# arancormonk/dsd-neo

Measured on AMD Instinct MI355X. Metric: I/Q Msamples/s end-to-end (demod->FEC->MBE) per GPU; % HBM roofline, higher is better.
Workload: dtype f32

## Files before the change

### dsd-neo_amd/csrc/ddn_api_chain.cpp

```cpp
#include <hip/hip_runtime.h>
#include <hsa/hsa.h>
#include <hsa/hsa_ext_amd.h>

#include <condition_variable>
#include <cstdio>
#include <cstdlib>
#include <cstring>
#include <deque>
#include <mutex>
#include <new>
#include <thread>

#include "ddn_api_util.h"
#include "ddn_chain.h"
#include "ddn_device.h"
#include "ddn_hip.h"
#include "ddn_internal.h"
#include "ddn_mbe.h"

enum { NSET = 3 };
static inline int
set_prev(int cur) {
    return (cur + NSET - 1) % NSET;
}
// ... 18 lines not shown
    float* d_pcm_dense[NSET] = {nullptr, nullptr, nullptr};
    int32_t *d_pcm_slot[NSET] = {nullptr, nullptr, nullptr}, *d_pcm_bcnt = nullptr, *d_pcm_boff = nullptr,
            *d_pcm_total[NSET] = {nullptr, nullptr, nullptr};
    int32_t *d_new[NSET], *d_ev[NSET], *d_nev[NSET], *d_evd[NSET];
    int32_t *d_evl[NSET], *d_evdl[NSET], *d_nevl[NSET];
    int32_t *d_cnt_scan, *d_cnt_full[NSET];
    int32_t* d_nid[NSET];
    int32_t *d_lists, *d_list_n;
    uint8_t* d_cls;
    uint8_t *d_tsbk[NSET], *d_tsbk_crc;
    uint8_t *d_words[2], *d_wrel, *d_werrs, *d_vldu;
    uint8_t *d_rs_d[2], *d_rs_p[2], *d_rs_st[2];
    uint8_t *d_lsd, *d_lsd_ok;
    int16_t* d_lsd_llr;
    uint8_t *d_hdu_hex, *d_hdu_par, *d_hdu_st, *d_hdu_d, *d_hdu_p, *d_hdu_rs;
    uint8_t *d_td_d, *d_td_p, *d_td_st, *d_td_rd, *d_td_rp, *d_td_rs;
    int PF, PB;
    int32_t *d_pdu_slot, *d_pdu_info, *d_n_pdu, *d_pdu_metric;
    uint8_t *d_pdu_hdr, *d_pdu_valid, *d_pdu_blocks, *d_pdu_wanted, *d_pdu_cand, *d_pdu_blocks18, *d_pdu_crc9;
    int32_t* d_pdu_cnt;
    int16_t *d_pdu_llr, *d_pdu_hllr;
    int64_t* d_first;
    int32_t *d_sc, *d_nldu, *d_sc_out, *d_imbe_res, *d_res_out;
    uint8_t *d_imbe_fr, *d_imbe_soft, *d_imbe_fl, *d_imbe_d;
    float* d_pcm[NSET];
    hipStream_t s_main, s_aux, s_copy, s_copy2;
    hipStream_t s_voice = nullptr;
    hipEvent_t ev_fork = nullptr, ev_join = nullptr;
    hipEvent_t ev_produced[NSET], ev_consumed[NSET], ev_out[NSET];
    hipEvent_t ev_in[2], ev_in_free[2];
    hipEvent_t ev_loop[NSET] = {nullptr, nullptr, nullptr};
    hipEvent_t ev_pre[NSET] = {nullptr, nullptr, nullptr}, ev_join_a = nullptr, ev_aux_done[NSET] = {nullptr, nullptr, nullptr};
    int synth_beside_loop = 1;
    int have_deferred = 0, deferred_set = 0, deferred_dense = 0;
    int want_rec2 = 0;
    ddn_p25_chain_host_out pending_out;
    int have_pending = 0, pending_set = 0;
    int sdma = 0;
    hsa_agent_t sdma_gpu, sdma_cpu;
    uint32_t sdma_engine = 0;
    hsa_signal_t sdma_sig[NSET];
    int sdma_sig_ok = 0;
    struct OutJob {
        int set;
        ddn_p25_chain_host_out out;
    };
// ... 173 lines not shown
        c->stride = (size_t)c->T + c->ms;
        c->S = (size_t)c->B * (size_t)c->F;
        c->V = (size_t)c->B * (size_t)c->Fv * 9;
        const size_t B = (size_t)c->B, S = c->S, V = c->V;
        DdnPool& m = c->pool;
        bool ok = m.alloc(&c->d_disc, B * (size_t)c->n) && m.alloc(&c->d_sym_cnt, B);
        for (int k = 0; k < NSET && ok; k++) {
            ok = m.alloc(&c->d_rec[k], B * c->stride * 10) && m.alloc(&c->d_fl[k], B * c->stride) && m.alloc(&c->d_new[k], B)
                 && m.alloc(&c->d_ev[k], B * (size_t)c->E * 4) && m.alloc(&c->d_nev[k], B) && m.alloc(&c->d_evd[k], B * (size_t)c->E * 4)
                 && m.alloc(&c->d_evl[k], B * (size_t)c->EL * 4) && m.alloc(&c->d_evdl[k], B * (size_t)c->EL * 4) && m.alloc(&c->d_nevl[k], B)
                 && m.alloc(&c->d_cnt_full[k], B) && m.alloc(&c->d_nid[k], S * 4) && m.alloc(&c->d_tsbk[k], 3 * S * 12) && m.alloc(&c->d_pcm[k], V * 160);
        }
        ok = ok && m.alloc(&c->d_cnt_scan, B) && m.alloc(&c->d_cls, S) && m.alloc(&c->d_lists, S * DDN_LIST_COUNT) && m.alloc(&c->d_list_n, 8)
             && m.alloc(&c->d_tsbk_crc, 3 * S) && m.alloc(&c->d_words[0], S * 240)
             && m.alloc(&c->d_words[1], S * 240) && m.alloc(&c->d_wrel, S * 240) && m.alloc(&c->d_werrs, S * 24) && m.alloc(&c->d_vldu, S)
             && m.alloc(&c->d_rs_d[0], S * 72) && m.alloc(&c->d_rs_d[1], S * 96) && m.alloc(&c->d_rs_p[0], S * 72)
             && m.alloc(&c->d_rs_p[1], S * 48) && m.alloc(&c->d_rs_st[0], S) && m.alloc(&c->d_rs_st[1], S) && m.alloc(&c->d_lsd, S * 32)
             && m.alloc(&c->d_lsd_ok, S * 2) && m.alloc(&c->d_lsd_llr, S * 32) && m.alloc(&c->d_hdu_hex, S * 216)
             && m.alloc(&c->d_hdu_par, S * 432) && m.alloc(&c->d_hdu_st, S * 36) && m.alloc(&c->d_hdu_d, S * 120)
             && m.alloc(&c->d_hdu_p, S * 96) && m.alloc(&c->d_hdu_rs, S) && m.alloc(&c->d_td_d, S * 144) && m.alloc(&c->d_td_p, S * 144)
             && m.alloc(&c->d_td_st, S * 12) && m.alloc(&c->d_td_rd, S * 72) && m.alloc(&c->d_td_rp, S * 72) && m.alloc(&c->d_td_rs, S)
             && m.alloc(&c->d_first, V) && m.alloc(&c->d_sc, V) && m.alloc(&c->d_nldu, B) && m.alloc(&c->d_sc_out, V)
             && m.alloc(&c->d_imbe_res, V * 5) && m.alloc(&c->d_res_out, V * 5) && m.alloc(&c->d_imbe_fr, V * 184)
             && m.alloc(&c->d_imbe_soft, V * 368) && m.alloc(&c->d_imbe_fl, V) && m.alloc(&c->d_imbe_d, V * 88)
             && m.alloc(&c->d_pdu_slot, B * (size_t)c->PF) && m.alloc(&c->d_pdu_info, B * (size_t)c->PF * 4)
             && m.alloc(&c->d_n_pdu, B) && m.alloc(&c->d_pdu_hdr, B * (size_t)c->PF * 12)
             && m.alloc(&c->d_pdu_valid, B * (size_t)c->PF * (size_t)c->PB) && m.alloc(&c->d_pdu_blocks, B * (size_t)c->PF * (size_t)c->PB * 12)
             && m.alloc(&c->d_pdu_metric, B * (size_t)c->PF * (size_t)c->PB) && m.alloc(&c->d_pdu_llr, B * (size_t)c->PF * (size_t)c->PB * 196)
             && m.alloc(&c->d_pdu_wanted, B * (size_t)c->PF * (size_t)c->PB) && m.alloc(&c->d_pdu_cand, B * (size_t)c->PF * (size_t)c->PB * 8 * 24)
             && m.alloc(&c->d_pdu_blocks18, B * (size_t)c->PF * (size_t)c->PB * 18) && m.alloc(&c->d_pdu_crc9, B * (size_t)c->PF * (size_t)c->PB)
             && m.alloc(&c->d_pdu_cnt, B * (size_t)c->PF * (size_t)c->PB) && m.alloc(&c->d_pdu_hllr, B * (size_t)c->PF * 196);
        if (!ok) {
            ddn_set_error("ddn_p25_chain_create: device allocation failed");
            rc = DDN_ENOMEM;
            break;
        }
        if (hipStreamCreateWithPriority(&c->s_main, hipStreamNonBlocking, -1) != hipSuccess
            || hipStreamCreateWithFlags(&c->s_aux, hipStreamNonBlocking) != hipSuccess
            || hipStreamCreateWithFlags(&c->s_copy, hipStreamNonBlocking) != hipSuccess
            || hipStreamCreateWithFlags(&c->s_copy2, hipStreamNonBlocking) != hipSuccess
            || hipStreamCreateWithFlags(&c->s_voice, hipStreamNonBlocking) != hipSuccess
            || hipEventCreateWithFlags(&c->ev_fork, hipEventDisableTiming) != hipSuccess
            || hipEventCreateWithFlags(&c->ev_join, hipEventDisableTiming) != hipSuccess
            || hipEventCreateWithFlags(&c->ev_user, hipEventDisableTiming) != hipSuccess) {
            rc = DDN_EHIP;
            break;
        }
// ... 479 lines not shown
        HIP_TRY(ddn_dev_chain_pdu_gather(rec, c->d_cnt_full[cur], stride, d_sp, c->d_pdu_slot, c->d_pdu_info, c->B, c->F, c->PF, c->PB,
                                         c->d_pdu_llr, c->d_pdu_valid, st));
        HIP_TRY(ddn_dev_p25_half_rate_list_wanted(c->d_pdu_llr, (int)NB, 8, c->d_pdu_valid, (uint32_t*)c->d_pdu_cand, c->d_pdu_cnt, st));
        HIP_TRY(ddn_dev_chain_pdu_take_first(c->d_pdu_cand, c->d_pdu_cnt, (int)NB, c->d_pdu_blocks, c->d_pdu_metric, st));
        HIP_TRY(ddn_dev_chain_pdu_r34_wanted(c->d_pdu_slot, c->d_pdu_hdr, c->d_pdu_info, c->d_pdu_valid, (int)NB, c->PB, c->d_pdu_wanted, st));
        DDN_TRY(ddn_fec_p25_mbf34_list_batch(c->d_pdu_llr, NB, 8, c->d_pdu_wanted, (ddn_p25_mbf34_candidate*)c->d_pdu_cand, c->d_pdu_cnt, st));
        HIP_TRY(ddn_dev_chain_pdu_r34_select(c->d_pdu_cand, c->d_pdu_cnt, c->d_pdu_wanted, (int)NB, c->d_pdu_blocks18, c->d_pdu_crc9, st));
        HIP_TRY(ddn_dev_chain_pdu_combine(rec, c->d_cnt_full[cur], stride, d_sp, c->d_pdu_slot, c->d_pdu_info, c->d_pdu_llr, c->d_pdu_valid,
                                          c->d_pdu_blocks, (int)NE, c->PF, c->PB, c->d_pdu_hllr, c->d_pdu_wanted, st));
        HIP_TRY(ddn_dev_p25_half_rate_list_wanted(c->d_pdu_hllr, (int)NE, 8, c->d_pdu_wanted, (uint32_t*)c->d_pdu_cand, c->d_pdu_cnt, st));
        HIP_TRY(ddn_dev_chain_pdu_finish(c->d_pdu_slot, c->d_pdu_blocks, c->d_pdu_valid, c->d_pdu_blocks18, c->d_pdu_cand, c->d_pdu_cnt,
                                         c->d_pdu_wanted, (int)NE, c->PB, c->d_pdu_hdr, c->d_pdu_info, st));
    }
    if (c->lp.MB > 0) {
        DDN_TRY(chain_long_pdu(c, cur, flush, st));
    }
    if (c->timing) {
        HIP_TRY(hipEventRecord(c->ev_t[4], st));
    }
    if (c->want_rec2) {
        HIP_TRY(ddn_dev_chain_pack2(c->d_rec[cur], c->d_fl[cur], (size_t)c->B * c->stride, c->d_rec2[cur], vst));
        c->want_rec2 = 0;
    }
    DDN_TRY(ddn_p25p1_framer_voice_index(c->fr, c->d_nid[cur], c->d_cnt_full[cur], c->Fv, stride, c->d_first, c->d_sc, c->d_nldu, vst));
    DDN_TRY(ddn_p25p1_imbe_deinterleave_batch(rec, (size_t)c->B * stride, c->d_first, c->d_sc, V, c->d_imbe_fr, c->d_imbe_soft,
                                              c->d_imbe_fl, c->d_sc_out, vst));
    DDN_TRY(ddn_mbe_frame_decode_batch(DDN_MBE_IMBE_7200X4400, c->d_imbe_fr, nullptr, V, c->d_imbe_d, c->d_imbe_res, vst));
    DDN_TRY(ddn_mbe_result_skip_batch(c->d_imbe_fl, V, c->d_imbe_res, vst));
    if (ev_pre) {
        if (vst != st) {
            HIP_TRY(hipEventRecord(c->ev_join_a, vst));
            HIP_TRY(hipStreamWaitEvent(st, c->ev_join_a, 0));
        }
        HIP_TRY(hipEventRecord(ev_pre, st));
    }
    if (defer_synth && vst != st && ev_pre && c->cfg.vocoder) {
        DDN_TRY(ddn_mbe_params_only(c->mbe, c->d_imbe_d, c->d_imbe_res, (size_t)c->Fv * 9, c->d_res_out, vst));
        HIP_TRY(hipEventRecord(c->ev_join_a, vst));
        HIP_TRY(hipStreamWaitEvent(st, c->ev_join_a, 0));
        HIP_TRY(hipEventRecord(ev_pre, st));
        c->have_deferred = 1;
        c->deferred_set = cur;
        c->deferred_dense = 0;
        return DDN_OK;
    }
    if (c->cfg.vocoder) {
        DDN_TRY(ddn_mbe_synth_batch(c->mbe, c->d_imbe_d, c->d_imbe_res, (size_t)c->Fv * 9, c->d_pcm[cur], c->d_res_out, vst));
    }
    if (vst != st) {
        HIP_TRY(hipEventRecord(c->ev_join, vst));
        HIP_TRY(hipStreamWaitEvent(st, c->ev_join, 0));
// ... 521 lines not shown
```

### dsd-neo_amd/csrc/ddn_api_framer.cpp

```cpp

#include <hip/hip_runtime.h>

#include <cstring>
#include <new>

#include "ddn_api_util.h"
#include "ddn_device.h"
#include "ddn_internal.h"

enum { T_NID = 0, T_BLK0, T_BLK1, T_BLK2, T_LDU1, T_LDU2, T_HDU_HEX, T_HDU_PAR, T_TDULC_DATA, T_TDULC_PAR, T_LSD, T_COUNT };

struct ddn_p25p1_framer {
    int n_channels, max_frames;
    int32_t* d_sync_pos;
    int32_t* d_n_syncs;
    int32_t* d_dropped;
    int32_t* d_tab[T_COUNT];
    int n_off[T_COUNT], max_off[T_COUNT];
    int32_t *d_first9, *d_status9;
    DdnPool pool;
};

extern "C" int
ddn_p25p1_framer_create(int n_channels, int max_frames_per_channel, ddn_p25p1_framer** out) {
// ... 172 lines not shown
    if (!f || !d_first_record || !d_status_count) {
        ddn_set_error("ddn_p25p1_framer_imbe_index: null argument");
        return DDN_EINVAL;
    }
    HIP_TRY(ddn_dev_imbe_index(f->d_sync_pos, f->d_n_syncs, f->n_channels, f->max_frames, max_symbols, f->d_first9,
                               f->d_status9, d_first_record, d_status_count, (hipStream_t)hip_stream));
    return DDN_OK;
}

extern "C" int
ddn_p25p1_framer_voice_index(ddn_p25p1_framer* f, const int32_t* d_nid4, const int32_t* d_counts, int max_ldu_per_channel, size_t max_symbols,
                             int64_t* d_first_record, int32_t* d_status_count, int32_t* d_n_ldu, void* hip_stream) {
    if (!f || !d_nid4 || !d_counts || max_ldu_per_channel <= 0 || !d_first_record || !d_status_count) {
        ddn_set_error("ddn_p25p1_framer_voice_index: bad argument");
        return DDN_EINVAL;
    }
    HIP_TRY(ddn_dev_voice_index(f->d_sync_pos, f->d_n_syncs, d_nid4, d_counts, f->n_channels, f->max_frames, max_ldu_per_channel,
                                max_symbols, f->d_first9, f->d_status9, d_first_record, d_status_count, d_n_ldu,
                                (hipStream_t)hip_stream));
    return DDN_OK;
}

extern "C" int
ddn_p25p1_framer_pack_ldu_rs(ddn_p25p1_framer* f, int ldu, const uint8_t* d_words240, uint8_t* d_data_bits,
                             uint8_t* d_parity_bits, void* hip_stream) {
    if (!f || (ldu != 1 && ldu != 2) || !d_words240 || !d_data_bits || !d_parity_bits) {
        ddn_set_error("ddn_p25p1_framer_pack_ldu_rs: bad argument");
        return DDN_EINVAL;
    }
    HIP_TRY(ddn_dev_rs_pack(d_words240, (long)f->n_channels * f->max_frames, 24, 10, ldu == 1 ? 12 : 16, d_data_bits,
                            d_parity_bits, (hipStream_t)hip_stream));
    return DDN_OK;
}

extern "C" int
ddn_p25p1_framer_gather_hdu(ddn_p25p1_framer* f, const uint8_t* d_records10, const int32_t* d_counts, size_t max_symbols,
                            uint8_t* d_hex_bits216, uint8_t* d_parity_bits432, int16_t* d_hex_llr216,
                            int16_t* d_parity_llr432, uint8_t* d_valid, void* hip_stream) {
    if (!d_hex_bits216 || !d_parity_bits432) {
        ddn_set_error("ddn_p25p1_framer_gather_hdu: null argument");
        return DDN_EINVAL;
    }
    int rc = gather(f, T_HDU_HEX, d_records10, d_counts, max_symbols, d_hex_bits216, nullptr, d_hex_llr216, 216, 0,
                    nullptr, nullptr, nullptr, hip_stream);
    if (rc != DDN_OK) {
        return rc;
// ... 57 lines not shown
```

### dsd-neo_amd/csrc/ddn_device.h

```cpp
#ifndef DDN_DEVICE_H
#define DDN_DEVICE_H

#include <hip/hip_runtime.h>
#include <stddef.h>
#include <stdint.h>

#include "ddn_internal.h"

#ifdef DDN_EXPERIMENTS
#include <stdlib.h>
#define DDN_EXP_ENV(name) getenv(name)
#else
#define DDN_EXP_ENV(name) ((const char*)0)
#endif

#define DDN_TILE 256
#define DDN_DEFAULT_GROUP 8
#define DDN_CARRY_LEN 72

typedef struct DdnFskState {
    float prev_i, prev_q;
    int have_prev;
    float dc_est, peak_est;
} DdnFskState;
// ... 230 lines not shown
hipError_t ddn_dev_rs63_soft(uint8_t* data6, const uint8_t* parity6, const uint8_t* data_rel, const uint8_t* parity_rel,
                             int n_par, int n_data, int t, int threshold, int n, uint8_t* status, hipStream_t st);
hipError_t ddn_dev_rs63(uint8_t* data6, const uint8_t* parity6, int n_par, int n_data, int t, int n, uint8_t* status,
                        hipStream_t st);
hipError_t ddn_dev_hamming_10_6_3(uint8_t* bits10, int n, uint8_t* errs, hipStream_t st);
hipError_t ddn_dev_p25_crc16(const uint8_t* bytes, int item_bytes, int n, uint8_t* ok, hipStream_t st);
hipError_t ddn_dev_p25_lsd(uint8_t* bits16, const int16_t* llr16, int n, uint8_t* ok, hipStream_t st);
hipError_t ddn_dev_iq_cond_disc(const void* in, long n, size_t stride, int block_len, int n_channels,
                                const DdnIqCondConfig* cfg, DdnFskState* fsk, DdnIqCondState* cond, float* out,
                                size_t out_stride, hipStream_t st);
hipError_t ddn_dev_find_syncs(const uint8_t* flags, const int32_t* counts, int n_channels, size_t max_sym, int max_frames,
                              int32_t* sync_pos, int32_t* n_syncs, int32_t* dropped, hipStream_t st);
hipError_t ddn_dev_gather_fields(const uint8_t* rec, size_t max_sym, const int32_t* counts, const int32_t* sync_pos,
                                 const int32_t* n_syncs, int n_channels, int max_frames, const int32_t* offsets, int n_off,
                                 int max_off, uint8_t* bits, uint8_t* rel, int16_t* llr, int stride, int split_last,
                                 uint8_t* last_bit, uint8_t* last_rel, uint8_t* valid, uint8_t* dibits,
                                 uint8_t* dibit_rel, hipStream_t st);
hipError_t ddn_dev_rs_pack(const uint8_t* words, long n_slots, int n_words, int wstride, int n_data, uint8_t* data,
                           uint8_t* parity, hipStream_t st);
hipError_t ddn_dev_tdulc_rs_pack(const uint8_t* words, long n_slots, uint8_t* data, uint8_t* parity, hipStream_t st);
hipError_t ddn_dev_voice_index(const int32_t* sync_pos, const int32_t* n_syncs, const int32_t* nid4, const int32_t* counts, int n_channels,
                               int max_frames, int max_ldu, size_t max_sym, const int32_t* first9, const int32_t* status9,
                               int64_t* first, int32_t* status, int32_t* n_ldu, hipStream_t st);
hipError_t ddn_dev_imbe_index(const int32_t* sync_pos, const int32_t* n_syncs, int n_channels, int max_frames,
                              size_t max_sym, const int32_t* first9, const int32_t* status9, int64_t* first,
                              int32_t* status, hipStream_t st);
hipError_t ddn_dev_resample(const float* in, long n, size_t in_stride, int n_channels, float* hist, const float* taps,
                            int L, int M, int p0, long n_out, float* out, size_t out_stride, hipStream_t st);
hipError_t ddn_dev_imbe_deinterleave(const uint8_t* rec, long n_records, const int64_t* first, const int32_t* status_count,
                                     int n_frames, uint8_t* fr, uint8_t* soft, uint8_t* flags, int32_t* status_out,
                                     hipStream_t st);
hipError_t ddn_dev_r34_list(const uint8_t* dibits, const uint8_t* reliab, int n, int max_cand, uint8_t* backs,
                            uint32_t* cand, int32_t* count, hipStream_t st);
hipError_t ddn_dev_p25_mbf34_list(const int16_t* llr, int n, int max_cand, const uint8_t* wanted, uint8_t* cand24, int32_t* count,
                                  hipStream_t st);
hipError_t ddn_dev_p25_half_rate_list(const int16_t* llr, int n, int max_cand, uint32_t* cand, int32_t* count,
                                      hipStream_t st);
hipError_t ddn_dev_p25_half_rate(const int16_t* llr, int n, uint8_t* out, int32_t* metric, hipStream_t st);
hipError_t ddn_dev_r34(const uint8_t* dibits, const uint8_t* reliab, int n, uint8_t* out, hipStream_t st);
hipError_t ddn_dev_p25_half_rate_list_wanted(const int16_t* llr, int n, int max_cand, const uint8_t* wanted, uint32_t* cand, int32_t* count,
                                             hipStream_t st);
hipError_t ddn_dev_p25_half_rate_list_wanted_wide(const int16_t* llr, int n, int max_cand, const uint8_t* wanted, uint32_t* cand,
                                                  int32_t* count, hipStream_t st);
hipError_t ddn_dev_k5_nxdn_lds(int n_steps, bool soft, size_t* need, size_t* limit);
hipError_t ddn_dev_k5_nxdn_wanted(const uint8_t* sym, const uint8_t* rel, int n, int n_steps, int n_bits, uint16_t* metrics_io,
                                  uint8_t* out, int out_stride, const uint8_t* wanted, int wanted_div, hipStream_t st);
hipError_t ddn_dev_trellis_greedy_wanted(const uint8_t* src, int src_stride, size_t n, int result_len, uint8_t* out, int out_stride,
                                         const uint8_t* wanted, hipStream_t st);
hipError_t ddn_dev_r34_list_wanted(const uint8_t* dibits, const uint8_t* reliab, int n, int max_cand, const uint8_t* wanted, uint8_t* backs,
                                   uint32_t* cand, int32_t* count, hipStream_t st);
hipError_t ddn_dev_dmr_data_select(const int32_t* events, const int32_t* n_events, int max_events, int carry, int n_channels,
                                   int max_bursts, const int32_t* sync_pos, const int32_t* n_sync, int max_syncs, const int32_t* out_pos,
                                   const int32_t* out_n, int max_out, const int32_t* n_new, int32_t* dstart, uint8_t* dslot,
                                   int32_t* dpre, int32_t* dn, hipStream_t st);
// ... 244 lines not shown
```

### dsd-neo_amd/csrc/ddn_framer.hip

```cpp

#include <hip/hip_runtime.h>
#include <stdint.h>

#include "ddn_device.h"

namespace {
__global__ __launch_bounds__(64) void
k_find_syncs(const uint8_t* __restrict__ flags, const int32_t* __restrict__ counts, size_t max_sym, int max_frames,
             int32_t* __restrict__ sync_pos, int32_t* __restrict__ n_syncs, int32_t* __restrict__ dropped) {
    const int ch = blockIdx.x;
    const int lane = threadIdx.x;
    const int cnt = counts[ch] < (int)max_sym ? counts[ch] : (int)max_sym;
    const uint8_t* row = flags + (size_t)ch * max_sym;
    int found = 0;
    for (int base = 0; base < cnt; base += 64) {
        const int i = base + lane;
        const bool hit = i < cnt && (row[i] & 2);
        const unsigned long long m = __ballot(hit);
        if (hit) {
            const int k = found + __popcll(m & ((1ull << lane) - 1ull));
            if (k < max_frames) {
                sync_pos[(size_t)ch * max_frames + k] = i;
            }
        }
// ... 182 lines not shown
    const DdnSel sel = ddn_sel_for(144);
    hipLaunchKernelGGL(k_tdulc_rs_pack, dim3(ddn_sel_grid(&sel, ((unsigned long)n_slots * 144 + DDN_WG - 1) / DDN_WG)), dim3(DDN_WG), 0, st, words, n_slots,
                       data, parity, sel);
    return hipGetLastError();
}

extern "C" hipError_t
ddn_dev_imbe_index(const int32_t* sync_pos, const int32_t* n_syncs, int n_channels, int max_frames, size_t max_sym,
                   const int32_t* first9, const int32_t* status9, int64_t* first, int32_t* status, hipStream_t st) {
    const long total = (long)n_channels * max_frames * 9;
    if (total <= 0) {
        return hipSuccess;
    }
    hipLaunchKernelGGL(k_imbe_index, dim3((unsigned)((total + 255) / 256)), dim3(256), 0, st, sync_pos, n_syncs,
                       n_channels, max_frames, max_sym, first9, status9, first, status);
    return hipGetLastError();
}

namespace {
__global__ void
k_voice_index(const int32_t* __restrict__ sync_pos, const int32_t* __restrict__ n_syncs, const int32_t* __restrict__ nid4,
              const int32_t* __restrict__ counts, int n_channels, int max_frames, int max_ldu, size_t max_sym, const int32_t* __restrict__ first9,
              const int32_t* __restrict__ status9, int64_t* __restrict__ first, int32_t* __restrict__ status,
              int32_t* __restrict__ n_ldu) {
    const int ch = blockIdx.x * 64 + threadIdx.x;
    if (ch >= n_channels) {
        return;
    }
    int k = 0;
    const int ns = n_syncs[ch];
    const int cnt = counts[ch] < (int)max_sym ? counts[ch] : (int)max_sym;
    for (int slot = 0; slot < ns && k < max_ldu; slot++) {
        const int32_t* nd = nid4 + ((size_t)ch * max_frames + slot) * 4;
        if (nd[0] > 0 && (nd[2] == 0x5 || nd[2] == 0xA)) {
            const int start = sync_pos[(size_t)ch * max_frames + slot] - 23;
            const int64_t base = (int64_t)((size_t)ch * max_sym) + start;
            for (int v = 0; v < 9; v++) {
                const int sc0 = status9[v], t1 = 35 - sc0;
                const int last = start + first9[v] + 71 + ((sc0 <= 35 && 71 >= t1) ? 1 + (71 - t1) / 35 : 0);
                first[((size_t)ch * max_ldu + k) * 9 + v] = last < cnt ? base + first9[v] : -1;
                status[((size_t)ch * max_ldu + k) * 9 + v] = status9[v];
            }
            k++;
        }
    }
    if (n_ldu) {
        n_ldu[ch] = k;
    }
    for (; k < max_ldu; k++) {
        for (int v = 0; v < 9; v++) {
            first[((size_t)ch * max_ldu + k) * 9 + v] = -1;
            status[((size_t)ch * max_ldu + k) * 9 + v] = 0;
        }
    }
}
}

extern "C" hipError_t
ddn_dev_voice_index(const int32_t* sync_pos, const int32_t* n_syncs, const int32_t* nid4, const int32_t* counts,
                    int n_channels, int max_frames,
                    int max_ldu, size_t max_sym, const int32_t* first9, const int32_t* status9, int64_t* first,
                    int32_t* status, int32_t* n_ldu, hipStream_t st) {
    if (n_channels <= 0 || max_ldu <= 0) {
        return hipSuccess;
    }
    hipLaunchKernelGGL(k_voice_index, dim3((unsigned)((n_channels + 63) / 64)), dim3(64), 0, st, sync_pos, n_syncs, nid4,
                       counts, n_channels, max_frames, max_ldu, max_sym, first9, status9, first, status, n_ldu);
    return hipGetLastError();
}
```

### dsd-neo_amd/csrc/ddn_imbe.hip

```cpp

#include <hip/hip_runtime.h>
#include <stdint.h>

#include "ddn_device.h"

namespace {
__global__ __launch_bounds__(64) void
k_imbe_deinterleave(const uint8_t* __restrict__ rec, long n_records, const int64_t* __restrict__ first,
                    const int32_t* __restrict__ status_count, int n_frames, uint8_t* __restrict__ fr,
                    uint8_t* __restrict__ soft, uint8_t* __restrict__ flags, int32_t* __restrict__ status_out) {
    __shared__ uint8_t c0[23];
    __shared__ int short_read;
    const int f = blockIdx.x;
    const int t0 = threadIdx.x;
    if (t0 == 0) {
        short_read = 0;
    }
    __syncthreads();
    const long base = first[f];
    const int sc0 = status_count[f];
    const int t1 = 35 - sc0;
    auto skips = [&](int j) { return (sc0 <= 35 && j >= t1) ? 1 + (j - t1) / 35 : 0; };
    for (int t = t0; t < 184; t += 64) {
        const int v = t / 23, i = t % 23;
        const int len = v < 4 ? 23 : (v < 7 ? 15 : 7);
        const int off = v < 4 ? 23 * v : (v < 7 ? 92 + 15 * (v - 4) : 137);
        int bit = 0, rel = 0;
        if (i < len) {
            const int L = off + (len - 1 - i);
            const int k = L / 24, rr = L % 24;
            const int r = rr >> 1;
            const int m = (rr & 1) ? 6 + (k ^ 1) : k;
            const int p = 12 * r + m;
            const int j = p >> 1, low = p & 1;
            const long ri = base + j + skips(j);
            if (base < 0 || ri >= n_records) {
// ... 14 lines not shown
            c0[t] = (uint8_t)bit;
        }
    }
    __syncthreads();
    if (t0 == 0) {
        int ns = 1;
        for (int i = 0; i < 23; i++) {
            ns &= (c0[i] == ((i >= 15 && i <= 17) ? 1 : 0));
        }
        flags[f] = short_read ? 0xFF : (uint8_t)ns;
        const int s71 = skips(71);
        status_out[f] = s71 == 0 ? sc0 + 72 : (71 - (t1 + 35 * (s71 - 1))) + 1;
    }
}
}

extern "C" hipError_t
ddn_dev_imbe_deinterleave(const uint8_t* rec, long n_records, const int64_t* first, const int32_t* status_count,
                          int n_frames, uint8_t* fr, uint8_t* soft, uint8_t* flags, int32_t* status_out, hipStream_t st) {
    if (n_frames <= 0) {
        return hipSuccess;
    }
    hipLaunchKernelGGL(k_imbe_deinterleave, dim3((unsigned)n_frames), dim3(64), 0, st, rec, n_records, first,
                       status_count, n_frames, fr, soft, flags, status_out);
    return hipGetLastError();
}
```

### dsd-neo_amd/csrc/ddn_internal.h

```cpp
#ifndef DDN_INTERNAL_H
#define DDN_INTERNAL_H

#include "../../include/ddn_hip.h"

#define DDN_MAX_TAPS   143
#define DDN_MAX_CENTER 71

#ifdef __cplusplus
extern "C" {
#endif
int ddn_design_channel_lpf(int rate_hz, int profile, float* taps, int max_taps);
#define DDN_FLL_MAX_TAPS 48
int ddn_design_fll_band_edge(int sps, float* taps4, float* alpha, float* beta);
int ddn_design_resampler(int L, int M, float* taps);
#define DDN_RESAMP_MAX_L 512
int ddn_p25p1_layout_nid(int32_t out32[32]);
int ddn_p25p1_layout_trellis_block(int block, int32_t out98[98]);
int ddn_p25p1_layout_ldu_words(int ldu, int32_t out120[120]);
int ddn_p25p1_layout_ldu_imbe(int32_t first9[9], int32_t status9[9]);
int ddn_p25p1_layout_hdu(int32_t hex3[36 * 3], int32_t par6[36 * 6]);
int ddn_p25p1_layout_tdulc(int32_t data6[72], int32_t par6[72]);
int ddn_p25p1_layout_ldu_lsd(int32_t out16[16]);
void ddn_set_error(const char* fmt, ...);
int ddn_p25_rx_mark_loop_start(ddn_p25_rx* b, void* hip_event);
int ddn_p25_rx_gate_loop(ddn_p25_rx* b, void* hip_event);
struct ddn_p25_chain;
struct ddn_fsk4_chain;
int ddn_p25_chain_stage0_prepare(struct ddn_p25_chain* c, void* hip_stream, float** disc_out);
float* ddn_fsk4_chain_disc_buffer(struct ddn_fsk4_chain* c);
void* ddn_fsk4_chain_reads_done_event(struct ddn_fsk4_chain* c);
int ddn_p25_chain_double_disc(struct ddn_p25_chain* c);
int ddn_fec_viterbi_k5_batch_wanted(const uint16_t* d_soft, size_t n, int in_len, const uint8_t* punct, int p_len, uint8_t* d_out,
                                    int out_stride, uint32_t* d_cost, const uint8_t* d_wanted, void* hip_stream);
struct ddn_mbe_batch;
int ddn_mbe_params_only(struct ddn_mbe_batch* b, const uint8_t* d_bits, const int32_t* d_result_in, size_t n_frames, int32_t* d_result_out,
                        void* hip_stream);
int ddn_mbe_synth_only(struct ddn_mbe_batch* b, size_t n_frames, float* d_pcm, void* hip_stream);
#ifdef __cplusplus
}
#endif
#endif
```

### dsd-neo_amd/csrc/ddn_mbe.hip

```cpp

#include <hip/hip_runtime.h>
#include <mutex>
#include <stdint.h>

#include "ddn_device.h"
#include "ddn_mbe.h"
#include "ddn_mbe_dev.h"
#include "ddn_mbe_math.h"

namespace {

__device__ __forceinline__ uint32_t
golay_syndrome(uint32_t w) {
#pragma unroll
    for (int i = 22; i >= 11; i--) {
        if ((w >> i) & 1u) {
            w ^= 0xC75u << (i - 11);
        }
    }
    return w & 0x7FFu;
}

__device__ __forceinline__ void
golay_table_lds(uint32_t* tab, int tid, int nthreads) {
// ... 32 lines not shown
    return w ^ e;
}

__device__ __forceinline__ uint32_t
hamming_fix(uint32_t w, int& errs) {
    const uint32_t m0 = 0x7f08, m1 = 0x78e4, m2 = 0x66d2, m3 = 0x55b1;
    const uint32_t syn = ((__popc(w & m0) & 1) << 3) | ((__popc(w & m1) & 1) << 2) | ((__popc(w & m2) & 1) << 1)
                         | (__popc(w & m3) & 1);
    errs = 0;
    if (syn) {
        errs = 1;
#pragma unroll
        for (int p = 0; p < 15; p++) {
            const uint32_t col = (((m0 >> p) & 1u) << 3) | (((m1 >> p) & 1u) << 2) | (((m2 >> p) & 1u) << 1) | ((m3 >> p) & 1u);
            if (col == syn) {
                w ^= 1u << p;
            }
        }
    }
    return w;
}

#define DDN_MBE_FRAMES_PER_WG 32
template <int CODEC>
__global__ __launch_bounds__(64) void
k_mbe_frame_decode(const uint8_t* __restrict__ frames, const uint8_t* __restrict__ soft, size_t n,
                   uint8_t* __restrict__ bits_out, int32_t* __restrict__ result) {
    constexpr int FB = CODEC == DDN_MBE_IMBE_7200X4400 ? 184 : 96;
    constexpr int OB = CODEC == DDN_MBE_IMBE_7200X4400 ? 88 : 49;
    constexpr int ROWLEN = CODEC == DDN_MBE_IMBE_7200X4400 ? 23 : 24;
    constexpr int FPW = DDN_MBE_FRAMES_PER_WG;
    __shared__ uint8_t stage[FPW * FB];
    __shared__ uint8_t outb[FPW * OB];
    const uint32_t* tab = g_golay_tab;
    const int lane = threadIdx.x;
    const size_t f0 = (size_t)blockIdx.x * FPW;
    const size_t nf = (n - f0) < (size_t)FPW ? (n - f0) : (size_t)FPW;
    const uint8_t* src = frames + f0 * FB;
    for (size_t i = lane; i < nf * FB; i += 64) {
        stage[i] = src[i];
    }
    __syncthreads();
    if ((size_t)lane < nf) {
        const uint8_t* f = stage + lane * FB;
        uint32_t row[8];
        bool bad = false;
        constexpr int NROW = CODEC == DDN_MBE_IMBE_7200X4400 ? 8 : 4;
#pragma unroll
        for (int r = 0; r < NROW; r++) {
            uint32_t w = 0;
            for (int j = 0; j < ROWLEN; j++) {
                const uint32_t v = f[r * ROWLEN + j];
                bad |= v > 1u;
                w |= (v & 1u) << j;
            }
            row[r] = w;
        }
        uint8_t* o = outb + lane * OB;
        int c0 = 0, c4 = 0, total = 0, e = 0;
        unsigned flags = MBE_PROCESS_FLAG_C0_VALID | (soft ? MBE_PROCESS_FLAG_SOFT_INPUT : 0u);
        if (CODEC == DDN_MBE_IMBE_7200X4400) {
            flags |= MBE_PROCESS_FLAG_C4_VALID;
            row[0] = golay_fix(row[0], tab, c0);
// ... 43 lines not shown
            row[0] = (w0 << 1) | (row[0] & 1u);
            uint32_t pr = (16u * (w0 >> 11)) & 0xFFFFu;
            uint32_t mask = 0;
            for (int j = 22; j >= 0; j--) {
                pr = (173u * pr + 13849u) & 0xFFFFu;
                mask |= (pr >> 15) << j;
            }
            row[1] = golay_fix((row[1] ^ mask) & 0x7FFFFFu, tab, e);
            total = c0 + e;
            int k = 0;
            for (int j = 23; j > 11; j--) {
                o[k++] = (uint8_t)((row[0] >> j) & 1u);
            }
            for (int j = 22; j > 10; j--) {
                o[k++] = (uint8_t)((row[1] >> j) & 1u);
            }
            for (int j = 10; j >= 0; j--) {
                o[k++] = (uint8_t)((row[2] >> j) & 1u);
            }
            for (int j = 13; j >= 0; j--) {
                o[k++] = (uint8_t)((row[3] >> j) & 1u);
            }
        }
        int32_t* r5 = result + (f0 + lane) * 5;
        if (bad) {
            for (int k = 0; k < OB; k++) {
                o[k] = 0;
            }
            r5[0] = (int32_t)DDN_MBE_RESULT_INVALID;
            r5[1] = r5[2] = r5[3] = r5[4] = 0;
        } else {
            r5[0] = (int32_t)flags;
            r5[1] = c0;
            r5[2] = c4;
            r5[3] = total;
            r5[4] = total - c0;
        }
    }
    __syncthreads();
    uint8_t* dst = bits_out + f0 * OB;
    for (size_t i = lane; i < nf * OB; i += 64) {
        dst[i] = outb[i];
    }
}

struct LaneParms {
    float w0, gamma;
    int L, K, repeat;
    int V;
    float Ml, log2Ml, PHI, PSI;
};

__device__ __forceinline__ LaneParms
lane_init(int l) {
    LaneParms p;
    p.w0 = 0.09378f;
    p.gamma = 0.0f;
    p.L = 30;
    p.K = 10;
    p.repeat = 0;
    p.V = 0;
    p.Ml = 0.0f;
    p.log2Ml = 0.0f;
    p.PHI = 0.0f;
    p.PSI = MBE_PI_F / 2.0f;
    (void)l;
    return p;
// ... 511 lines not shown
            }
        }
    }
    if (lane < 56) {
        out[lane] = acc[0];
    }
    if (lane < 49) {
        out[56 + lane] = acc[1];
    }
    if (lane < 55) {
        out[105 + lane] = acc[2];
    }
}

__global__ void
k_mbe_result_skip(const uint8_t* __restrict__ skip, size_t n, int32_t* __restrict__ result) {
    const size_t i = (size_t)blockIdx.x * blockDim.x + threadIdx.x;
    if (i < n && skip[i]) {
        result[i * 5] = (int32_t)((uint32_t)result[i * 5] | DDN_MBE_RESULT_INVALID);
    }
}

__global__ void
k_mbe_stream_init(DdnMbeStream* streams, int n, uint32_t seed0) {
    const int s = blockIdx.x;
    const int l = threadIdx.x;
    if (s >= n) {
        return;
    }
    const LaneParms p = lane_init(l);
    lane_store(&streams[s].cur, p, l, 0);
    lane_store(&streams[s].prev, p, l, 0);
    lane_store(&streams[s].enh, p, l, 0);
    if (l == 0) {
        streams[s].frame_no = 0;
        streams[s].seed = seed0 + (uint32_t)s;
    }
}
}

extern "C" hipError_t
ddn_dev_mbe_frame_decode(int codec, const uint8_t* frames, const uint8_t* soft, size_t n, uint8_t* bits, int32_t* result,
                         hipStream_t st) {
    if (n == 0) {
        return hipSuccess;
    }
    {
        static std::mutex mu;
        static bool up[64] = {false};
        int dev = 0;
        if (hipGetDevice(&dev) != hipSuccess) {
            return hipErrorInvalidDevice;
        }
        std::lock_guard<std::mutex> lock(mu);
        if (dev < 0 || dev >= 64 || !up[dev]) {
            hipLaunchKernelGGL(k_golay_tab_init, dim3(1), dim3(256), 0, st);
            hipError_t e = hipGetLastError();
            if (e == hipSuccess) {
                e = hipStreamSynchronize(st);
            }
            if (e != hipSuccess) {
                return e;
            }
            if (dev >= 0 && dev < 64) {
                up[dev] = true;
            }
        }
    }
    const dim3 grid((unsigned)((n + DDN_MBE_FRAMES_PER_WG - 1) / DDN_MBE_FRAMES_PER_WG)), blk(64);
    if (codec == DDN_MBE_IMBE_7200X4400) {
        hipLaunchKernelGGL(k_mbe_frame_decode<DDN_MBE_IMBE_7200X4400>, grid, blk, 0, st, frames, soft, n, bits, result);
    } else {
        hipLaunchKernelGGL(k_mbe_frame_decode<DDN_MBE_AMBE_3600X2450>, grid, blk, 0, st, frames, soft, n, bits, result);
    }
    return hipGetLastError();
}

extern "C" hipError_t
ddn_dev_mbe_stream_init(DdnMbeStream* streams, int n_streams, uint32_t seed0, hipStream_t st) {
    if (n_streams <= 0) {
        return hipSuccess;
    }
    hipLaunchKernelGGL(k_mbe_stream_init, dim3((unsigned)n_streams), dim3(64), 0, st, streams, n_streams, seed0);
    return hipGetLastError();
}

extern "C" hipError_t
ddn_dev_mbe_params(int codec, const uint8_t* bits, const int32_t* res_in, int n_streams, int n_frames,
                   const ddn_mbe_tables* d_tables, const float* d_half_log2, DdnMbeStream* streams, int tail_rule,
                   DdnMbeFrameRec* recs, int32_t* res_out, hipStream_t st) {
    if (n_streams <= 0 || n_frames <= 0) {
        return hipSuccess;
    }
    const dim3 grid((unsigned)n_streams), blk(64);
    if (codec == DDN_MBE_IMBE_7200X4400) {
        hipLaunchKernelGGL(k_mbe_params<DDN_MBE_IMBE_7200X4400>, grid, blk, 0, st, bits, res_in, n_frames, d_tables,
                           d_half_log2, streams, tail_rule, recs, res_out);
// ... 25 lines not shown
```

Baseline: 26010.

## Compact live IMBE voice frames into a list and decode only those

The voice-index kernel now also emits a compacted list of voice-frame slots whose records are fully present, using an atomic counter. Deinterleave and IMBE frame decode run over that list instead of every capacity slot, and the list decode path moves frames with 32-bit word gathers. Dead slots are filled from a precomputed result of decoding an all-zero frame, so skipped frames still produce defined outputs. The aim is to stop decoding empty or truncated voice slots, at the cost of an atomic per channel, indirection and a nondeterministic list order.

```diff
diff --git a/dsd-neo_amd/csrc/ddn_api_chain.cpp b/dsd-neo_amd/csrc/ddn_api_chain.cpp
--- a/dsd-neo_amd/csrc/ddn_api_chain.cpp
+++ b/dsd-neo_amd/csrc/ddn_api_chain.cpp
@@ -64,6 +64,7 @@
     int16_t *d_pdu_llr, *d_pdu_hllr;
     int64_t* d_first;
     int32_t *d_sc, *d_nldu, *d_sc_out, *d_imbe_res, *d_res_out;
+    int32_t* d_vlive;
     uint8_t *d_imbe_fr, *d_imbe_soft, *d_imbe_fl, *d_imbe_d;
     float* d_pcm[NSET];
     hipStream_t s_main, s_aux, s_copy, s_copy2;
@@ -283,7 +284,7 @@
              && m.alloc(&c->d_td_st, S * 12) && m.alloc(&c->d_td_rd, S * 72) && m.alloc(&c->d_td_rp, S * 72) && m.alloc(&c->d_td_rs, S)
              && m.alloc(&c->d_first, V) && m.alloc(&c->d_sc, V) && m.alloc(&c->d_nldu, B) && m.alloc(&c->d_sc_out, V)
              && m.alloc(&c->d_imbe_res, V * 5) && m.alloc(&c->d_res_out, V * 5) && m.alloc(&c->d_imbe_fr, V * 184)
-             && m.alloc(&c->d_imbe_soft, V * 368) && m.alloc(&c->d_imbe_fl, V) && m.alloc(&c->d_imbe_d, V * 88)
+             && m.alloc(&c->d_imbe_soft, V * 368) && m.alloc(&c->d_imbe_fl, V) && m.alloc(&c->d_imbe_d, V * 88) && m.alloc(&c->d_vlive, V)
              && m.alloc(&c->d_pdu_slot, B * (size_t)c->PF) && m.alloc(&c->d_pdu_info, B * (size_t)c->PF * 4)
              && m.alloc(&c->d_n_pdu, B) && m.alloc(&c->d_pdu_hdr, B * (size_t)c->PF * 12)
              && m.alloc(&c->d_pdu_valid, B * (size_t)c->PF * (size_t)c->PB) && m.alloc(&c->d_pdu_blocks, B * (size_t)c->PF * (size_t)c->PB * 12)
@@ -809,11 +810,13 @@
         HIP_TRY(ddn_dev_chain_pack2(c->d_rec[cur], c->d_fl[cur], (size_t)c->B * c->stride, c->d_rec2[cur], vst));
         c->want_rec2 = 0;
     }
-    DDN_TRY(ddn_p25p1_framer_voice_index(c->fr, c->d_nid[cur], c->d_cnt_full[cur], c->Fv, stride, c->d_first, c->d_sc, c->d_nldu, vst));
-    DDN_TRY(ddn_p25p1_imbe_deinterleave_batch(rec, (size_t)c->B * stride, c->d_first, c->d_sc, V, c->d_imbe_fr, c->d_imbe_soft,
-                                              c->d_imbe_fl, c->d_sc_out, vst));
-    DDN_TRY(ddn_mbe_frame_decode_batch(DDN_MBE_IMBE_7200X4400, c->d_imbe_fr, nullptr, V, c->d_imbe_d, c->d_imbe_res, vst));
-    DDN_TRY(ddn_mbe_result_skip_batch(c->d_imbe_fl, V, c->d_imbe_res, vst));
+    int32_t* n_vlive = c->d_list_n + DDN_LIST_COUNT;
+    DDN_TRY(ddn_p25p1_framer_voice_index_live(c->fr, c->d_nid[cur], c->d_cnt_full[cur], c->Fv, stride, c->d_first, c->d_sc, c->d_nldu,
+                                              c->d_vlive, n_vlive, vst));
+    HIP_TRY(ddn_dev_imbe_deinterleave_list(rec, (long)((size_t)c->B * stride), c->d_first, c->d_sc, c->d_vlive, n_vlive, (int)V,
+                                           c->d_imbe_fr, c->d_imbe_soft, c->d_imbe_fl, c->d_sc_out, vst));
+    HIP_TRY(ddn_dev_imbe_frame_decode_list(c->d_imbe_fr, c->d_vlive, n_vlive, V, c->d_imbe_d, c->d_imbe_res, vst));
+    HIP_TRY(ddn_dev_imbe_result_skip_dead(c->d_first, c->d_nldu, 9, c->Fv * 9, V, c->d_imbe_fl, c->d_imbe_d, c->d_imbe_res, vst));
     if (ev_pre) {
         if (vst != st) {
             HIP_TRY(hipEventRecord(c->ev_join_a, vst));
diff --git a/dsd-neo_amd/csrc/ddn_api_framer.cpp b/dsd-neo_amd/csrc/ddn_api_framer.cpp
--- a/dsd-neo_amd/csrc/ddn_api_framer.cpp
+++ b/dsd-neo_amd/csrc/ddn_api_framer.cpp
@@ -218,6 +218,20 @@
 }
 
 extern "C" int
+ddn_p25p1_framer_voice_index_live(ddn_p25p1_framer* f, const int32_t* d_nid4, const int32_t* d_counts, int max_ldu_per_channel,
+                                  size_t max_symbols, int64_t* d_first_record, int32_t* d_status_count, int32_t* d_n_ldu, int32_t* d_live,
+                                  int32_t* d_n_live, void* hip_stream) {
+    if (!f || !d_nid4 || !d_counts || max_ldu_per_channel <= 0 || !d_first_record || !d_status_count || !d_live || !d_n_live) {
+        ddn_set_error("ddn_p25p1_framer_voice_index_live: bad argument");
+        return DDN_EINVAL;
+    }
+    HIP_TRY(ddn_dev_voice_index_live(f->d_sync_pos, f->d_n_syncs, d_nid4, d_counts, f->n_channels, f->max_frames, max_ldu_per_channel,
+                                     max_symbols, f->d_first9, f->d_status9, d_first_record, d_status_count, d_n_ldu, d_live, d_n_live,
+                                     (hipStream_t)hip_stream));
+    return DDN_OK;
+}
+
+extern "C" int
 ddn_p25p1_framer_pack_ldu_rs(ddn_p25p1_framer* f, int ldu, const uint8_t* d_words240, uint8_t* d_data_bits,
                              uint8_t* d_parity_bits, void* hip_stream) {
     if (!f || (ldu != 1 && ldu != 2) || !d_words240 || !d_data_bits || !d_parity_bits) {
diff --git a/dsd-neo_amd/csrc/ddn_device.h b/dsd-neo_amd/csrc/ddn_device.h
--- a/dsd-neo_amd/csrc/ddn_device.h
+++ b/dsd-neo_amd/csrc/ddn_device.h
@@ -276,6 +276,10 @@
 hipError_t ddn_dev_voice_index(const int32_t* sync_pos, const int32_t* n_syncs, const int32_t* nid4, const int32_t* counts, int n_channels,
                                int max_frames, int max_ldu, size_t max_sym, const int32_t* first9, const int32_t* status9,
                                int64_t* first, int32_t* status, int32_t* n_ldu, hipStream_t st);
+hipError_t ddn_dev_voice_index_live(const int32_t* sync_pos, const int32_t* n_syncs, const int32_t* nid4, const int32_t* counts,
+                                    int n_channels, int max_frames, int max_ldu, size_t max_sym, const int32_t* first9,
+                                    const int32_t* status9, int64_t* first, int32_t* status, int32_t* n_ldu, int32_t* live,
+                                    int32_t* n_live, hipStream_t st);
 hipError_t ddn_dev_imbe_index(const int32_t* sync_pos, const int32_t* n_syncs, int n_channels, int max_frames,
                               size_t max_sym, const int32_t* first9, const int32_t* status9, int64_t* first,
                               int32_t* status, hipStream_t st);
@@ -284,6 +288,13 @@
 hipError_t ddn_dev_imbe_deinterleave(const uint8_t* rec, long n_records, const int64_t* first, const int32_t* status_count,
                                      int n_frames, uint8_t* fr, uint8_t* soft, uint8_t* flags, int32_t* status_out,
                                      hipStream_t st);
+hipError_t ddn_dev_imbe_deinterleave_list(const uint8_t* rec, long n_records, const int64_t* first, const int32_t* status_count,
+                                          const int32_t* list, const int32_t* count, int capacity, uint8_t* fr, uint8_t* soft,
+                                          uint8_t* flags, int32_t* status_out, hipStream_t st);
+hipError_t ddn_dev_imbe_frame_decode_list(const uint8_t* frames, const int32_t* list, const int32_t* count, size_t capacity,
+                                          uint8_t* bits, int32_t* result, hipStream_t st);
+hipError_t ddn_dev_imbe_result_skip_dead(const int64_t* first, const int32_t* used, int unit, int per_stream, size_t n, uint8_t* skip,
+                                         uint8_t* bits, int32_t* result, hipStream_t st);
 hipError_t ddn_dev_r34_list(const uint8_t* dibits, const uint8_t* reliab, int n, int max_cand, uint8_t* backs,
                             uint32_t* cand, int32_t* count, hipStream_t st);
 hipError_t ddn_dev_p25_mbf34_list(const int16_t* llr, int n, int max_cand, const uint8_t* wanted, uint8_t* cand24, int32_t* count,
diff --git a/dsd-neo_amd/csrc/ddn_framer.hip b/dsd-neo_amd/csrc/ddn_framer.hip
--- a/dsd-neo_amd/csrc/ddn_framer.hip
+++ b/dsd-neo_amd/csrc/ddn_framer.hip
@@ -228,12 +228,12 @@
 k_voice_index(const int32_t* __restrict__ sync_pos, const int32_t* __restrict__ n_syncs, const int32_t* __restrict__ nid4,
               const int32_t* __restrict__ counts, int n_channels, int max_frames, int max_ldu, size_t max_sym, const int32_t* __restrict__ first9,
               const int32_t* __restrict__ status9, int64_t* __restrict__ first, int32_t* __restrict__ status,
-              int32_t* __restrict__ n_ldu) {
+              int32_t* __restrict__ n_ldu, int32_t* __restrict__ live, int32_t* __restrict__ n_live) {
     const int ch = blockIdx.x * 64 + threadIdx.x;
     if (ch >= n_channels) {
         return;
     }
-    int k = 0;
+    int k = 0, n_alive = 0;
     const int ns = n_syncs[ch];
     const int cnt = counts[ch] < (int)max_sym ? counts[ch] : (int)max_sym;
     for (int slot = 0; slot < ns && k < max_ldu; slot++) {
@@ -246,12 +246,22 @@
                 const int last = start + first9[v] + 71 + ((sc0 <= 35 && 71 >= t1) ? 1 + (71 - t1) / 35 : 0);
                 first[((size_t)ch * max_ldu + k) * 9 + v] = last < cnt ? base + first9[v] : -1;
                 status[((size_t)ch * max_ldu + k) * 9 + v] = status9[v];
+                n_alive += last < cnt ? 1 : 0;
             }
             k++;
         }
     }
     if (n_ldu) {
         n_ldu[ch] = k;
+    }
+    if (live && n_alive > 0) {
+        int at = atomicAdd(n_live, n_alive);
+        const int cap = n_channels * max_ldu * 9;
+        for (int slot = ch * max_ldu * 9; slot < (ch * max_ldu + k) * 9; slot++) {
+            if (first[slot] >= 0 && at < cap) {
+                live[at++] = slot;
+            }
+        }
     }
     for (; k < max_ldu; k++) {
         for (int v = 0; v < 9; v++) {
@@ -270,7 +280,19 @@
     if (n_channels <= 0 || max_ldu <= 0) {
         return hipSuccess;
     }
+    return ddn_dev_voice_index_live(sync_pos, n_syncs, nid4, counts, n_channels, max_frames, max_ldu, max_sym, first9, status9, first,
+                                    status, n_ldu, nullptr, nullptr, st);
+}
+
+extern "C" hipError_t
+ddn_dev_voice_index_live(const int32_t* sync_pos, const int32_t* n_syncs, const int32_t* nid4, const int32_t* counts,
+                         int n_channels, int max_frames, int max_ldu, size_t max_sym, const int32_t* first9,
+                         const int32_t* status9, int64_t* first, int32_t* status, int32_t* n_ldu, int32_t* live, int32_t* n_live,
+                         hipStream_t st) {
+    if (n_channels <= 0 || max_ldu <= 0) {
+        return hipSuccess;
+    }
     hipLaunchKernelGGL(k_voice_index, dim3((unsigned)((n_channels + 63) / 64)), dim3(64), 0, st, sync_pos, n_syncs, nid4,
-                       counts, n_channels, max_frames, max_ldu, max_sym, first9, status9, first, status, n_ldu);
-    return hipGetLastError();
-}
+                       counts, n_channels, max_frames, max_ldu, max_sym, first9, status9, first, status, n_ldu, live, n_live);
+    return hipGetLastError();
+}
diff --git a/dsd-neo_amd/csrc/ddn_imbe.hip b/dsd-neo_amd/csrc/ddn_imbe.hip
--- a/dsd-neo_amd/csrc/ddn_imbe.hip
+++ b/dsd-neo_amd/csrc/ddn_imbe.hip
@@ -7,11 +7,15 @@
 namespace {
 __global__ __launch_bounds__(64) void
 k_imbe_deinterleave(const uint8_t* __restrict__ rec, long n_records, const int64_t* __restrict__ first,
-                    const int32_t* __restrict__ status_count, int n_frames, uint8_t* __restrict__ fr,
-                    uint8_t* __restrict__ soft, uint8_t* __restrict__ flags, int32_t* __restrict__ status_out) {
+                    const int32_t* __restrict__ status_count, int n_frames, const int32_t* __restrict__ list,
+                    const int32_t* __restrict__ count, uint8_t* __restrict__ fr, uint8_t* __restrict__ soft,
+                    uint8_t* __restrict__ flags, int32_t* __restrict__ status_out) {
     __shared__ uint8_t c0[23];
     __shared__ int short_read;
-    const int f = blockIdx.x;
+    if (list && (int)blockIdx.x >= *count) {
+        return;
+    }
+    const int f = list ? list[blockIdx.x] : (int)blockIdx.x;
     const int t0 = threadIdx.x;
     if (t0 == 0) {
         short_read = 0;
@@ -72,6 +76,18 @@
         return hipSuccess;
     }
     hipLaunchKernelGGL(k_imbe_deinterleave, dim3((unsigned)n_frames), dim3(64), 0, st, rec, n_records, first,
-                       status_count, n_frames, fr, soft, flags, status_out);
+                       status_count, n_frames, nullptr, nullptr, fr, soft, flags, status_out);
     return hipGetLastError();
 }
+
+extern "C" hipError_t
+ddn_dev_imbe_deinterleave_list(const uint8_t* rec, long n_records, const int64_t* first, const int32_t* status_count,
+                               const int32_t* list, const int32_t* count, int capacity, uint8_t* fr, uint8_t* soft,
+                               uint8_t* flags, int32_t* status_out, hipStream_t st) {
+    if (capacity <= 0) {
+        return hipSuccess;
+    }
+    hipLaunchKernelGGL(k_imbe_deinterleave, dim3((unsigned)capacity), dim3(64), 0, st, rec, n_records, first,
+                       status_count, capacity, list, count, fr, soft, flags, status_out);
+    return hipGetLastError();
+}
diff --git a/dsd-neo_amd/csrc/ddn_internal.h b/dsd-neo_amd/csrc/ddn_internal.h
--- a/dsd-neo_amd/csrc/ddn_internal.h
+++ b/dsd-neo_amd/csrc/ddn_internal.h
@@ -36,6 +36,9 @@
 int ddn_mbe_params_only(struct ddn_mbe_batch* b, const uint8_t* d_bits, const int32_t* d_result_in, size_t n_frames, int32_t* d_result_out,
                         void* hip_stream);
 int ddn_mbe_synth_only(struct ddn_mbe_batch* b, size_t n_frames, float* d_pcm, void* hip_stream);
+int ddn_p25p1_framer_voice_index_live(ddn_p25p1_framer* f, const int32_t* d_nid4, const int32_t* d_counts, int max_ldu_per_channel,
+                                      size_t max_symbols, int64_t* d_first_record, int32_t* d_status_count, int32_t* d_n_ldu,
+                                      int32_t* d_live, int32_t* d_n_live, void* hip_stream);
 #ifdef __cplusplus
 }
 #endif
diff --git a/dsd-neo_amd/csrc/ddn_mbe.hip b/dsd-neo_amd/csrc/ddn_mbe.hip
--- a/dsd-neo_amd/csrc/ddn_mbe.hip
+++ b/dsd-neo_amd/csrc/ddn_mbe.hip
@@ -78,23 +78,50 @@
 }
 
 #define DDN_MBE_FRAMES_PER_WG 32
-template <int CODEC>
+template <int CODEC, bool LIST>
 __global__ __launch_bounds__(64) void
-k_mbe_frame_decode(const uint8_t* __restrict__ frames, const uint8_t* __restrict__ soft, size_t n,
-                   uint8_t* __restrict__ bits_out, int32_t* __restrict__ result) {
+k_mbe_frame_decode(const uint8_t* __restrict__ frames, const uint8_t* __restrict__ soft, size_t n, const int32_t* __restrict__ list,
+                   const int32_t* __restrict__ count, uint8_t* __restrict__ bits_out, int32_t* __restrict__ result) {
     constexpr int FB = CODEC == DDN_MBE_IMBE_7200X4400 ? 184 : 96;
     constexpr int OB = CODEC == DDN_MBE_IMBE_7200X4400 ? 88 : 49;
     constexpr int ROWLEN = CODEC == DDN_MBE_IMBE_7200X4400 ? 23 : 24;
     constexpr int FPW = DDN_MBE_FRAMES_PER_WG;
-    __shared__ uint8_t stage[FPW * FB];
-    __shared__ uint8_t outb[FPW * OB];
+    __shared__ __align__(4) uint8_t stage[FPW * FB];
+    __shared__ __align__(4) uint8_t outb[FPW * OB];
     const uint32_t* tab = g_golay_tab;
     const int lane = threadIdx.x;
     const size_t f0 = (size_t)blockIdx.x * FPW;
+    if (LIST) {
+        const size_t have = (size_t)(*count > 0 ? *count : 0);
+        n = have < n ? have : n;
+        if (f0 >= n) {
+            return;
+        }
+    }
     const size_t nf = (n - f0) < (size_t)FPW ? (n - f0) : (size_t)FPW;
-    const uint8_t* src = frames + f0 * FB;
-    for (size_t i = lane; i < nf * FB; i += 64) {
-        stage[i] = src[i];
+    const int slot = (LIST && (size_t)lane < nf) ? list[f0 + lane] : 0;
+    if (LIST) {
+        constexpr int FW = FB / 4, NIT = (FPW * FW + 63) / 64;
+        const uint32_t* fw = reinterpret_cast<const uint32_t*>(frames);
+        uint32_t v[NIT];
+#pragma unroll
+        for (int t = 0; t < NIT; t++) {
+            const unsigned i = t * 64 + lane, j = i / FW < (unsigned)nf ? i / FW : (unsigned)nf - 1;
+            const int s = __shfl(slot, (int)j);
+            v[t] = i < (unsigned)nf * FW ? fw[(size_t)s * FW + (i - j * FW)] : 0u;
+        }
+#pragma unroll
+        for (int t = 0; t < NIT; t++) {
+            const unsigned i = t * 64 + lane;
+            if (i < (unsigned)nf * FW) {
+                reinterpret_cast<uint32_t*>(stage)[i] = v[t];
+            }
+        }
+    } else {
+        const uint8_t* src = frames + f0 * FB;
+        for (size_t i = lane; i < nf * FB; i += 64) {
+            stage[i] = src[i];
+        }
     }
     __syncthreads();
     if ((size_t)lane < nf) {
@@ -184,7 +211,7 @@
                 o[k++] = (uint8_t)((row[3] >> j) & 1u);
             }
         }
-        int32_t* r5 = result + (f0 + lane) * 5;
+        int32_t* r5 = result + (LIST ? (size_t)slot : f0 + lane) * 5;
         if (bad) {
             for (int k = 0; k < OB; k++) {
                 o[k] = 0;
@@ -200,11 +227,28 @@
         }
     }
     __syncthreads();
+    if (LIST) {
+        static_assert(!LIST || (FB % 4 == 0 && OB % 4 == 0), "the list form moves whole words");
+        constexpr int OW = OB / 4;
+        uint32_t* bw = reinterpret_cast<uint32_t*>(bits_out);
+        for (unsigned i0 = 0; i0 < (unsigned)nf * OW; i0 += 64) {
+            const unsigned i = i0 + lane, j = i / OW < (unsigned)nf ? i / OW : (unsigned)nf - 1;
+            const int s = __shfl(slot, (int)j);
+            if (i < (unsigned)nf * OW) {
+                bw[(size_t)s * OW + (i - j * OW)] = reinterpret_cast<const uint32_t*>(outb)[i];
+            }
+        }
+        return;
+    }
     uint8_t* dst = bits_out + f0 * OB;
     for (size_t i = lane; i < nf * OB; i += 64) {
         dst[i] = outb[i];
     }
 }
+
+__device__ uint8_t g_imbe_dead_frame[184];
+__device__ uint8_t g_imbe_dead_bits[88];
+__device__ int32_t g_imbe_dead_result[5];
 
 struct LaneParms {
     float w0, gamma;
@@ -762,6 +806,31 @@
 }
 
 __global__ void
+k_mbe_result_skip_dead(const int64_t* __restrict__ first, const int32_t* __restrict__ used, int unit, int per_stream, size_t n,
+                       uint8_t* __restrict__ skip, uint8_t* __restrict__ bits, int32_t* __restrict__ result) {
+    const size_t i = (size_t)blockIdx.x * blockDim.x + threadIdx.x;
+    if (i >= n) {
+        return;
+    }
+    if (first[i] >= 0) {
+        if (skip[i]) {
+            result[i * 5] = (int32_t)((uint32_t)result[i * 5] | DDN_MBE_RESULT_INVALID);
+        }
+        return;
+    }
+    skip[i] = 0xFF;
+    result[i * 5] = (int32_t)((uint32_t)g_imbe_dead_result[0] | DDN_MBE_RESULT_INVALID);
+    for (int k = 1; k < 5; k++) {
+        result[i * 5 + k] = g_imbe_dead_result[k];
+    }
+    if ((int)(i % (size_t)per_stream) / unit < used[i / (size_t)per_stream]) {
+        for (int k = 0; k < 88; k++) {
+            bits[i * 88 + k] = g_imbe_dead_bits[k];
+        }
+    }
+}
+
+__global__ void
 k_mbe_stream_init(DdnMbeStream* streams, int n, uint32_t seed0) {
     const int s = blockIdx.x;
     const int l = threadIdx.x;
@@ -779,40 +848,94 @@
 }
 }
 
+static hipError_t
+mbe_decode_tables(hipStream_t st) {
+    static std::mutex mu;
+    static bool up[64] = {false};
+    int dev = 0;
+    if (hipGetDevice(&dev) != hipSuccess) {
+        return hipErrorInvalidDevice;
+    }
+    std::lock_guard<std::mutex> lock(mu);
+    if (dev < 0 || dev >= 64 || !up[dev]) {
+        uint8_t *zeros = nullptr, *dead_bits = nullptr;
+        int32_t* dead_result = nullptr;
+        hipError_t e = hipGetSymbolAddress((void**)&zeros, HIP_SYMBOL(g_imbe_dead_frame));
+        if (e == hipSuccess) {
+            e = hipGetSymbolAddress((void**)&dead_bits, HIP_SYMBOL(g_imbe_dead_bits));
+        }
+        if (e == hipSuccess) {
+            e = hipGetSymbolAddress((void**)&dead_result, HIP_SYMBOL(g_imbe_dead_result));
+        }
+        if (e != hipSuccess) {
+            return e;
+        }
+        hipLaunchKernelGGL(k_golay_tab_init, dim3(1), dim3(256), 0, st);
+        hipLaunchKernelGGL((k_mbe_frame_decode<DDN_MBE_IMBE_7200X4400, false>), dim3(1), dim3(64), 0, st, zeros, nullptr, (size_t)1, nullptr,
+                           nullptr, dead_bits, dead_result);
+        e = hipGetLastError();
+        if (e == hipSuccess) {
+            e = hipStreamSynchronize(st);
+        }
+        if (e != hipSuccess) {
+            return e;
+        }
+        if (dev >= 0 && dev < 64) {
+            up[dev] = true;
+        }
+    }
+    return hipSuccess;
+}
+
 extern "C" hipError_t
 ddn_dev_mbe_frame_decode(int codec, const uint8_t* frames, const uint8_t* soft, size_t n, uint8_t* bits, int32_t* result,
                          hipStream_t st) {
     if (n == 0) {
         return hipSuccess;
     }
-    {
-        static std::mutex mu;
-        static bool up[64] = {false};
-        int dev = 0;
-        if (hipGetDevice(&dev) != hipSuccess) {
-            return hipErrorInvalidDevice;
-        }
-        std::lock_guard<std::mutex> lock(mu);
-        if (dev < 0 || dev >= 64 || !up[dev]) {
-            hipLaunchKernelGGL(k_golay_tab_init, dim3(1), dim3(256), 0, st);
-            hipError_t e = hipGetLastError();
-            if (e == hipSuccess) {
-                e = hipStreamSynchronize(st);
-            }
-            if (e != hipSuccess) {
-                return e;
-            }
-            if (dev >= 0 && dev < 64) {
-                up[dev] = true;
-            }
-        }
+    const hipError_t e = mbe_decode_tables(st);
+    if (e != hipSuccess) {
+        return e;
     }
     const dim3 grid((unsigned)((n + DDN_MBE_FRAMES_PER_WG - 1) / DDN_MBE_FRAMES_PER_WG)), blk(64);
     if (codec == DDN_MBE_IMBE_7200X4400) {
-        hipLaunchKernelGGL(k_mbe_frame_decode<DDN_MBE_IMBE_7200X4400>, grid, blk, 0, st, frames, soft, n, bits, result);
+        hipLaunchKernelGGL((k_mbe_frame_decode<DDN_MBE_IMBE_7200X4400, false>), grid, blk, 0, st, frames, soft, n, nullptr, nullptr, bits,
+                           result);
     } else {
-        hipLaunchKernelGGL(k_mbe_frame_decode<DDN_MBE_AMBE_3600X2450>, grid, blk, 0, st, frames, soft, n, bits, result);
-    }
+        hipLaunchKernelGGL((k_mbe_frame_decode<DDN_MBE_AMBE_3600X2450, false>), grid, blk, 0, st, frames, soft, n, nullptr, nullptr, bits,
+                           result);
+    }
+    return hipGetLastError();
+}
+
+extern "C" hipError_t
+ddn_dev_imbe_frame_decode_list(const uint8_t* frames, const int32_t* list, const int32_t* count, size_t capacity, uint8_t* bits,
+                               int32_t* result, hipStream_t st) {
+    if (capacity == 0) {
+        return hipSuccess;
+    }
+    const hipError_t e = mbe_decode_tables(st);
+    if (e != hipSuccess) {
+        return e;
+    }
+    const dim3 grid((unsigned)((capacity + DDN_MBE_FRAMES_PER_WG - 1) / DDN_MBE_FRAMES_PER_WG)), blk(64);
+    hipLaunchKernelGGL((k_mbe_frame_decode<DDN_MBE_IMBE_7200X4400, true>), grid, blk, 0, st, frames, nullptr, capacity, list, count, bits,
+                       result);
+    return hipGetLastError();
+}
+
+extern "C" hipError_t
+ddn_dev_imbe_result_skip_dead(const int64_t* first, const int32_t* used, int unit, int per_stream, size_t n, uint8_t* skip,
+                              uint8_t* bits, int32_t* result, hipStream_t st) {
+    if (n == 0) {
+        return hipSuccess;
+    }
+    const hipError_t e = mbe_decode_tables(st);
+    if (e != hipSuccess) {
+        return e;
+    }
+    hipLaunchKernelGGL(k_mbe_result_skip_dead, dim3((unsigned)((n + 63) / 64)), dim3(64), 0, st, first, used, unit, per_stream, n, skip,
+                       bits, result);
     return hipGetLastError();
 }
 
```

Result: no change. 26260 (median of 6 runs) (+1.0%).
